# PlayVoice/whisper-vits-svc

Hardware: AMD Instinct MI355X
Metric: audio-seconds/sec end-to-end SVC @32kHz, 10s clips (Whisper-PPG -> flow -> NSF-BigVGAN) (higher is better)
Workload: dtype f32; 1 GPU; configs[1]: batch=1 x 10s clip per GPU, whisper-large-v2 dims (24 of 32 encoder blocks) + base.yaml prior/flow/NSF-BigVGAN; Whisper fp32, synthesizer fp32; clips_in_flight=4, gemm_ring2_mask=12, world_size=1, rccl_ranks_seen=1, whisper_weights_wire=f32, weights=packed on this rank

## Files before the change

whisper-vits-svc_amd/csrc/amp_fused.hip:

```cpp
#include "svcmi_rt.h"
#include "../../include/svcmi.h"

namespace {

constexpr int TPB = 256;
constexpr int RT = 8;
constexpr int CO = 10;
constexpr int DMAX = 5;

#include "snake_math.h"

template <int CP>
__device__ __forceinline__ int tile_row_offset(int t) {
    static_assert(CP == 12 || CP == 20 || CP == 40, "widths of the fused kernels");
    return CP == 12 ? (t << 3) + (t << 2) : CP == 20 ? (t << 4) + (t << 2) : (t << 5) + (t << 3);
}
__device__ __forceinline__ const float* tile_column(const float* xc) {
#ifndef SVCMI_EMU
    asm("" : "+v"(xc));
#endif
    return xc;
}
template <int CP>
__device__ __forceinline__ float tile_x(const float* xc, int t, int n, int ld) {
// ... 7 lines not shown
static inline bool tile_len_ok(int len, int ld) { return (long long)len * ld < (1LL << 31); }

struct AmpArgs {
    const float* x; const float* w; const float* bias; const float* res; float* y;
    const float* alpha_log; const float* beta_log; const float* filt;
    int n, ld, ldw, dil, accumulate, ks;
    float alpha;
};

template <bool H16, int LS>
__device__ __forceinline__ void tile_store(float* S, int row, int ch, float v) {
    if constexpr (H16) reinterpret_cast<unsigned short*>(S)[row * LS + ch] = (unsigned short)svcmi_cvt_pk_f16(v, 0.f);
    else S[row * LS + ch] = v;
}

template <int CP, int CR, int LS, bool H16 = false>
__device__ __forceinline__ void snake_tile(float* S, const float* xb, const float* alpha_log, const float* beta_log,
                                           const float* filt, int n, int ld, int t_blk, int halo, int rows, int tid) {
    struct { const float* alpha_log; const float* beta_log; const float* filt; } p = {alpha_log, beta_log, filt};
        float f[12];
#pragma unroll
        for (int k = 0; k < 12; ++k) f[k] = p.filt[k];
        const int runs = (rows + RT - 1) / RT;
        for (int item = tid; item < runs * CP; item += TPB) {
            const int ch = item % CP, run = item / CP;
            const int r0 = run * RT;
            const int t0 = t_blk - halo + r0;
            float out[RT];
            if (ch >= CR || t0 + RT <= 0 || t0 >= n) {
#pragma unroll
                for (int r = 0; r < RT; ++r) out[r] = 0.f;
            } else {
                const float a = expf(p.alpha_log[ch]);
                const float inv_b = 1.0f / (expf(p.beta_log[ch]) + 1e-9f);
                const float* xc = tile_column(xb + ch);
                SnakeWindow<RT + 10> xw;
#pragma unroll
                for (int i = 0; i < RT + 10; ++i) xw.set(i, tile_x<CP>(xc, t0 - 5 + i, n, ld));
                snake_run<RT>(xw, f, a, inv_b, xc, ld, n, t0, out);
#pragma unroll
                for (int r = 0; r < RT; ++r) {
                    const int t = t0 + r;
                    if (t < 0 || t >= n) out[r] = 0.f;
                }
            }
#pragma unroll
            for (int r = 0; r < RT; ++r)
                if (r0 + r < rows) tile_store<H16, LS>(S, r0 + r, ch, out[r]);
        }
}

template <int CP>
struct UTile {
    static constexpr int LU = 2 * CP + 2;
    __device__ __forceinline__ static int pos(int m) { return m * LU; }
    static constexpr int floats(int pair_rows) { return (pair_rows + 7) * LU; }
};

template <int CP, int CR, int LS, int MAXI, bool H16 = false>
__device__ __forceinline__ void snake_tile_u(float* smem, const float* xb, const float* alpha_log, const float* beta_log,
                                             const float* filt, int n, int ld, int t_blk, int halo, int rows, int tid) {
    constexpr int LU = UTile<CP>::LU;
    float f[12];
#pragma unroll
    for (int k = 0; k < 12; ++k) f[k] = filt[k];
    const int t_lo = t_blk - halo;
    const int pairs = rows + 5;
    const int mruns = (pairs + RT - 1) / RT;
    for (int item = tid; item < mruns * CP; item += TPB) {
        const int ch = item % CP, run = item / CP;
        if (ch >= CR) continue;
        const int m0 = run * RT, tq0 = t_lo + m0;
        svcmi_f32x2 s2[RT];
        if (2 * tq0 - 5 + 2 * RT - 1 < -12 || 2 * tq0 - 5 > 2 * n - 1 + 12) {
#pragma unroll
            for (int m = 0; m < RT; ++m) s2[m] = svcmi_splat2(0.f);
        } else {
            const float a = expf(alpha_log[ch]);
            const float inv_b = 1.0f / (expf(beta_log[ch]) + 1e-9f);
            const float* xc = tile_column(xb + ch);
            SnakeWindow<RT + 5> xw;
#pragma unroll
            for (int i = 0; i < RT + 5; ++i) xw.set(i, tile_x<CP>(xc, tq0 - 5 + i, n, ld));
            snake_pairs<RT>(xw, f, a, inv_b, xc, ld, n, tq0, s2);
        }
#pragma unroll
        for (int m = 0; m < RT; ++m)
            if (m0 + m < pairs) *reinterpret_cast<float2*>(smem + UTile<CP>::pos(m0 + m) + 2 * ch) = make_float2(s2[m][0], s2[m][1]);
    }
    __syncthreads();
    const int runs = (rows + RT - 1) / RT;
    float outs[MAXI][RT];
#pragma unroll
    for (int q = 0; q < MAXI; ++q) {
        const int item = tid + q * TPB;
        if (item < runs * CP) {
            const int ch = item % CP, run = item / CP, r0 = run * RT, t0 = t_lo + r0;
            if (ch >= CR || t0 + RT <= 0 || t0 >= n) {
#pragma unroll
                for (int r = 0; r < RT; ++r) outs[q][r] = 0.f;
            } else {
                svcmi_f32x2 P[RT + 5];
                const float* ub = smem + UTile<CP>::pos(r0) + 2 * ch;
#pragma unroll
                for (int i = 0; i < RT + 5; ++i) {
                    const float2 v = *reinterpret_cast<const float2*>(ub + i * LU);
                    P[i] = svcmi_f32x2{v.x, v.y};
                }
                snake_fir<RT>(P, f, outs[q]);
#pragma unroll
                for (int r = 0; r < RT; ++r) {
                    const int t = t0 + r;
                    if (t < 0 || t >= n) outs[q][r] = 0.f;
                }
            }
        }
    }
    __syncthreads();
#pragma unroll
    for (int q = 0; q < MAXI; ++q) {
        const int item = tid + q * TPB;
        if (item < runs * CP) {
            const int ch = item % CP, r0 = (item / CP) * RT;
#pragma unroll
            for (int r = 0; r < RT; ++r)
                if (r0 + r < rows) tile_store<H16, LS>(smem, r0 + r, ch, outs[q][r]);
        }
    }
}

template <int CP, int G, int TT, int KS>
struct AmpTile {
    static constexpr int TSUB = 4 / G;
    static constexpr int TB = TSUB * 64 * TT;
    static constexpr int LS = (CP / 4) % 2 ? CP : CP + 4;
    static constexpr int ROWS = TB + (KS - 1) * DMAX;
};

template <int CP, int CR, int KS_T, int G, int TT, bool UT = false>
__device__ __forceinline__ void snake_conv_body(const AmpArgs& p, float* S) {
    using TL = AmpTile<CP, G, TT, KS_T ? KS_T : 11>;
    const int KS = KS_T ? KS_T : p.ks;
    constexpr int TSUB = TL::TSUB, TB = TL::TB, LS = TL::LS;
    static_assert(G * CO >= CR && CP % 4 == 0 && CP >= CR, "channel split");

    const int tid = threadIdx.x, lane = tid & 63;
    const int wave = SVCMI_UNIFORM((int)(tid >> 6));
    const int b = blockIdx.y;
    const int n = p.n, ld = p.ld, d = p.dil;
    const int halo = (KS - 1) * d / 2;
    const int t_blk = blockIdx.x * TB;
    const int rows = TB + 2 * halo;
    const float* xb = p.x + (long long)b * n * ld;

    if constexpr (UT) snake_tile_u<CP, CR, LS, (((TL::ROWS + RT - 1) / RT) * CP + TPB - 1) / TPB>(S, xb, p.alpha_log, p.beta_log, p.filt, n, ld, t_blk, halo, rows, tid);
    else snake_tile<CP, CR, LS>(S, xb, p.alpha_log, p.beta_log, p.filt, n, ld, t_blk, halo, rows, tid);
    __syncthreads();

    const int g = wave % G, tsub = wave / G;
// ... 49 lines not shown
                }
            }
        }
    }

    float* yb = p.y + (long long)b * n * ld;
#pragma unroll
    for (int j = 0; j < TT; ++j) {
        const int t = t_blk + tl0 + 64 * j;
        if (t >= n) continue;
        float* yr = yb + (long long)t * ld + co0;
#pragma unroll
        for (int c = 0; c < NCO; c += 2) {
            float v0 = acc[j][c / 2][0], v1 = acc[j][c / 2][1];
            if (co0 + c >= CR) { v0 = 0.f; v1 = 0.f; }
            else {
                if (rb) {
                    float2 r2;
                    if constexpr (PRE) r2 = rpre[j][c / 2];
                    else r2 = *reinterpret_cast<const float2*>(rb + (long long)t * ld + co0 + c);
                    v0 += r2.x; v1 += r2.y;
                }
                v0 *= p.alpha; v1 *= p.alpha;
                if (p.accumulate) { const float2 o2 = *reinterpret_cast<const float2*>(yr + c); v0 += o2.x; v1 += o2.y; }
            }
            *reinterpret_cast<float2*>(yr + c) = make_float2(v0, v1);
        }
        if (g == G - 1) {
#pragma unroll
            for (int c = G * CO; c < CP; c += 2) *reinterpret_cast<float2*>(yb + (long long)t * ld + c) = make_float2(0.f, 0.f);
        }
    }
}

template <int CP, int CR, int KS, int G, int TT>
__global__ __launch_bounds__(TPB) void snake_conv_kernel(AmpArgs p) {
    using TL = AmpTile<CP, G, TT, KS>;
    __shared__ __attribute__((aligned(16))) float S[TL::ROWS * TL::LS];
    snake_conv_body<CP, CR, KS, G, TT>(p, S);
}

constexpr int AMP_GROUP = 3;
struct AmpGroupArgs {
    AmpArgs p[AMP_GROUP];
};

template <int CP, int CR, int G, int TT>
__global__ __launch_bounds__(TPB) void snake_conv_group_kernel(AmpGroupArgs g) {
    using TL = AmpTile<CP, G, TT, 11>;
    __shared__ __attribute__((aligned(16))) float S[TL::ROWS * TL::LS];
    snake_conv_body<CP, CR, 0, G, TT>(g.p[blockIdx.z], S);
}

template <int CP, int CR, int G, int TT>
__global__ __launch_bounds__(TPB) void snake_conv_group_u_kernel(AmpGroupArgs g) {
    using TL = AmpTile<CP, G, TT, 11>;
    constexpr int NU = UTile<CP>::floats(TL::ROWS + 5), NS = TL::ROWS * TL::LS;
    static_assert(((TL::ROWS + RT - 1) / RT) * CP <= 4 * TPB, "snake_tile_u keeps at most 4 work items per thread in registers");
    __shared__ __attribute__((aligned(16))) float S[NU > NS ? NU : NS];
    snake_conv_body<CP, CR, 0, G, TT, true>(g.p[blockIdx.z], S);
}

template <int CP, int CR, int TERMS>
struct Amp16 {
    static constexpr int CK = (CR + 7) / 8;
    static constexpr int LSH = 24;
    static constexpr int NCT = (CR + 15) / 16;
    static constexpr int TB = 256;
    static constexpr int ROWS = TB + 10 * DMAX;
    static constexpr int MAXSTEPS = (11 * CK + 3) / 4;
    static constexpr int S_FLOATS = (ROWS * LSH / 2 + 3) / 4 * 4;
    static constexpr int U_FLOATS = (UTile<CP>::floats(ROWS + 5) + 3) / 4 * 4;
    static constexpr int W_FLOATS = MAXSTEPS * NCT * TERMS * 64 * 4;
    static_assert(CK * 8 <= LSH && CP <= CK * 8 && CP + 4 >= CK * 8, "pad columns [CP, 8 CK) are one 8-byte store per row");
};

template <int CP, int CR, int TERMS, bool UT>
__device__ __forceinline__ void snake_conv16_body(const AmpArgs& p, float* smem, float* wl) {
    using TL = Amp16<CP, CR, TERMS>;
    constexpr int CK = TL::CK, LSH = TL::LSH, NCT = TL::NCT, TB = TL::TB;
    const int KS = p.ks;
    const int tid = threadIdx.x, lane = tid & 63;
    const int wave = SVCMI_UNIFORM((int)(tid >> 6));
    const int b = blockIdx.y;
    const int n = p.n, ld = p.ld, d = p.dil;
    const int halo = (KS - 1) * d / 2;
    const int t_blk = blockIdx.x * TB;
    const int rows = TB + 2 * halo;
    const float* xb = p.x + (long long)b * n * ld;
    const int nsteps = (KS * CK + 3) / 4;

    svcmi_u32x4* wf = reinterpret_cast<svcmi_u32x4*>(wl);
    auto pack_weights = [&] {
    for (int u = tid; u < nsteps * NCT * 64; u += TPB) {
        const int l = u & 63, f = u >> 6;
        const int ct = f % NCT, step = f / NCT;
        const int co = ct * 16 + (l & 15), s = 4 * step + (l >> 4);
        const int tap = s / CK, cb = s - tap * CK;
        float v[8];
#pragma unroll
        for (int h = 0; h < 2; ++h) {
            const int ci0 = cb * 8 + 4 * h;
            float4 q = make_float4(0.f, 0.f, 0.f, 0.f);
            if (co < CR && tap < KS && ci0 < CR) q = *reinterpret_cast<const float4*>(p.w + (long long)co * p.ldw + tap * CP + ci0);
            v[4 * h] = q.x;
            v[4 * h + 1] = ci0 + 1 < CR ? q.y : 0.f;
            v[4 * h + 2] = ci0 + 2 < CR ? q.z : 0.f;
            v[4 * h + 3] = ci0 + 3 < CR ? q.w : 0.f;
// ... 544 lines not shown
```

whisper-vits-svc_amd/csrc/conv_gemm_body.h:

```cpp
#pragma once
#include <type_traits>

#include "svcmi_rt.h"
#include "../../include/svcmi.h"

namespace {

#ifndef SVCMI_GEMM_MIDBAR
#define SVCMI_GEMM_MIDBAR 1
#endif
#ifndef SVCMI_GEMM_SPREAD
#define SVCMI_GEMM_SPREAD 1
#endif
#ifndef SVCMI_PROBE_NOMFMA
#define SVCMI_PROBE_NOMFMA 0
#endif
#ifndef SVCMI_PROBE_KTRACE
#define SVCMI_PROBE_KTRACE 0
#endif
#if SVCMI_PROBE_KTRACE
#ifndef SVCMI_PROBE_KTRACE_N
#define SVCMI_PROBE_KTRACE_N 0
#endif
constexpr unsigned TL_CAP = 1u << 22;
__device__ unsigned long long g_tl[5ull * TL_CAP];
__device__ unsigned g_tl_n;
__device__ unsigned long long g_ktrace[4 * 4 * 8192 + 8];
#endif
#ifndef SVCMI_GEMM_SPREAD2
#define SVCMI_GEMM_SPREAD2 1
#endif
constexpr int BK = 32;
enum { MODE_CHUNK = 0, MODE_VEC = 1, MODE_SCALAR = 2, MODE_CHUNK_RS = 3 };

enum { PREC_F32 = 0, PREC_BF16X3 = 1, PREC_BF16 = 2, PREC_F16 = 3, PREC_BF16_A16 = 4, PREC_F16_A16 = 5, PREC_BF16X3_A16 = 6, PREC_F16W2_A16 = 9 };

struct ConvArgs {
    const float* x; const float* w; const float* bias; const float* res; float* y; const int32_t* lengths;
    float* ws;
    int* cnt;
    long long x_bs, y_bs, r_bs;
    int t_in, t_out, c_in, ldx, n_out, ldw, ldy, ldr;
    int ksize, stride, dil, pad, rshift, act, flags;
    const unsigned short* w16;
    int ldw16;
    unsigned short* y16;
    long long y16_bs;
    int ldy16, y16_f16;
    int vec;
    int ktot;
    int split;
    int mt, nt;
    unsigned magic;
    float alpha;
};

__device__ __forceinline__ float act_apply(float v, int act) {
    switch (act) {
        case SVCMI_ACT_RELU: return v > 0.f ? v : 0.f;
        case SVCMI_ACT_GELU: return svcmi_gelu(v);
        case SVCMI_ACT_MISH: {
            float sp = v;
            if (!(v > 20.f)) {
                const float e = expf(v), u = 1.0f + e;
                sp = u == 1.0f ? e : logf(u) * (e / (u - 1.0f));
            }
            return v * tanhf(sp);
        }
        case SVCMI_ACT_TANH: return tanhf(v);
        case SVCMI_ACT_SIGMOID: return 1.0f / (1.0f + expf(-v));
        default: return v;
    }
}

__device__ __forceinline__ float epilogue(const ConvArgs& p, float v, float bias, const float* res_row, float* dst,
                                          int n, bool masked) {
    v = act_apply(v + bias, p.act);
    if (res_row) v += res_row[n];
    v *= p.alpha;
    if (p.flags & SVCMI_CONV_ACCUMULATE) v += *dst;
    return masked ? 0.f : v;
}

__device__ __forceinline__ int div_magic(int q, unsigned magic) {
    return magic ? (int)__umulhi((unsigned)q, magic) : q;
}

__device__ __forceinline__ int swz(int row) { return (row >> 1) & 7; }
__device__ __forceinline__ int swz16(int row) { return (0x78 >> (((row >> 2) & 3) * 2)) & 3; }

constexpr unsigned OOB = 0x40000000u;

template <int WM, int WN, int MODE, bool P16, int NSTO = 0, int PREC = PREC_F32, int NW = 4>
__device__ __forceinline__ void conv_gemm_body(const ConvArgs& p, const int grid_blocks, const int block_id) {
    static_assert(NW == 4 || (NW == 8 && P16 && PREC == PREC_F32), "eight-wave blocks: fp32 16x16x4 policy only");
    constexpr int NT = 64 * NW;
    constexpr bool A16 = PREC >= PREC_BF16_A16;
    constexpr bool LP = PREC != PREC_F32 && !A16;
    constexpr int KS = A16 ? 2 * BK : BK;
    constexpr unsigned ESZ = A16 ? 2u : 4u;
    constexpr bool F16OP = PREC == PREC_F16 || PREC == PREC_F16_A16 || PREC == PREC_F16W2_A16;
    constexpr bool X3A = PREC == PREC_BF16X3_A16;
    constexpr bool W2A = PREC == PREC_F16W2_A16;
    constexpr int NB = (PREC == PREC_BF16X3 || X3A || W2A) ? 2 : 1;
    constexpr int NA = X3A ? 2 : 1;
    constexpr int BM = P16 ? 16 * WM * NW : 64 * WM, BN = P16 ? 16 * WN : 64 * WN;
    constexpr int BROW = LP ? BK / 2 : BK;
    constexpr int BNL = LP ? (BN + 63) / 64 * 64 : (BN + 8 * NW - 1) / (8 * NW) * (8 * NW);
    constexpr int A_PER = BM / (8 * NW), B_PER = LP ? BNL / 64 : BNL / (8 * NW);
    constexpr int BTILE = BNL * BROW;
    constexpr int CLD = BN;
    constexpr int NST = NSTO ? NSTO : NW == 8 ? 3 : (X3A || (W2A && P16)) ? 2 : (LP ? 3 : (P16 ? ((BM + BNL) > 192 ? 2 : 3) : ((WM * WN == 1) ? 3 : (WM * WN == 2 ? 3 : 2))));
    constexpr int RING = NST * (NA * BM * BK + NB * BTILE);
    static_assert(LP || A16 || BM * CLD <= RING, "C tile must fit in the operand buffers");
    constexpr int BIAS0 = (RING > BM * CLD ? RING : BM * CLD) + 4, BIASN = (BN + 63) / 64 * 64;
    __shared__ __attribute__((aligned(16))) float smem[BIAS0 + BIASN];
    float* const As0 = smem;
    float* const Bs0 = smem + NST * NA * BM * BK;

#if SVCMI_PROBE_KTRACE
    unsigned long long kt_entry, tl_entry;
    asm volatile("s_memtime %0\n\ts_memrealtime %1\n\ts_waitcnt lgkmcnt(0)" : "=s"(kt_entry), "=s"(tl_entry));
#endif
    const int tid = threadIdx.x, lane = tid & 63;
    const int wave = SVCMI_UNIFORM((int)(tid >> 6));
    const int wm = P16 ? wave : (wave >> 1), wn = P16 ? 0 : (wave & 1);
    int bx, by, bz;
    {
        const int total = grid_blocks, id = block_id;
        const int q8 = total >> 3, r8 = total & 7, xcd = id & 7, slot = id >> 3;
        const int L = (xcd < r8 ? xcd * (q8 + 1) : r8 * (q8 + 1) + (xcd - r8) * q8) + slot;
        bx = L % p.mt;
        const int rest = L / p.mt;
        by = rest % p.nt;
        bz = rest / p.nt;
    }
    const int b = bz / p.split, slice = bz - b * p.split;
    const int m0 = bx * BM, n0 = by * BN;
    const int len = p.lengths ? p.lengths[b] : 0x7fffffff;
    const int t_lim = (p.flags & SVCMI_CONV_MASK_IN) ? (len < p.t_in ? len : p.t_in) : p.t_in;
    const int x_rows = (t_lim + (1 << p.rshift) - 1) >> p.rshift;
    const svcmi_rsrc xr = A16 ? svcmi_make_rsrc(reinterpret_cast<const unsigned short*>(p.x) + (long long)b * p.x_bs, (unsigned)x_rows * (unsigned)p.ldx * 2u)
                              : svcmi_make_rsrc(p.x + (long long)b * p.x_bs, (unsigned)x_rows * (unsigned)p.ldx * 4u);
    const svcmi_rsrc wr = (LP || A16) ? svcmi_make_rsrc(p.w16, (unsigned)p.n_out * (unsigned)(NB * p.ldw16) * 2u)
                             : svcmi_make_rsrc(p.w, (unsigned)p.n_out * (unsigned)p.ldw * 4u);

    const int nk_all = (p.ktot + KS - 1) / KS;
    const int it_beg = (int)((long long)nk_all * slice / p.split);
    const int it_end = (int)((long long)nk_all * (slice + 1) / p.split);

    const int prow = lane >> 3;
    const int lkq = ((lane & 7) ^ swz(prow + 8 * wave)) * 4;
    int a_tb[A_PER];
    unsigned a_row[A_PER];
    unsigned b_row[B_PER];
#pragma unroll
    for (int i = 0; i < A_PER; ++i) {
        const int t = m0 + (wave + NW * i) * 8 + prow;
        a_tb[i] = t * p.stride - p.pad;
        a_row[i] = t < p.t_out ? (unsigned)a_tb[i] * (unsigned)p.ldx * ESZ : OOB;
        if (t >= p.t_out) a_tb[i] = -0x40000000;
    }
#pragma unroll
    for (int i = 0; i < B_PER; ++i) {
        const int nl = (wave + NW * i) * (LP ? 16 : 8) + (LP ? (lane >> 2) : prow), n = n0 + nl;
        b_row[i] = (n < p.n_out && nl < BN) ? ((LP || A16) ? (unsigned)(n * NB * p.ldw16) * 2u : (unsigned)(n * p.ldw) * 4u) : OOB;
    }
    const int lkq16 = ((lane & 3) ^ swz16(lane >> 2)) * 16;
    int tap_u = 0, ci_u = 0;
// ... 95 lines not shown
#pragma unroll
        for (int i = 1; i < FA; ++i) svcmi_lds_landed(a4[i]);
#pragma unroll
        for (int j = 0; j < FB; ++j) svcmi_lds_landed(b4[j]);
    };
    auto load_frags_lp = [&](const float* Ab, const float* Bb, int s, svcmi_f32x4 (&a8)[WM][2], svcmi_f32x4 (&b8)[NB][WN], svcmi_f32x4& tie) {
        const int q = (P16 ? 0 : 2 * s) + fhi;
        const int pa = (q ^ swz(frow)) << 2, pb = (q ^ swz16(frow)) << 2;
#pragma unroll
        for (int i = 0; i < WM; ++i) {
            svcmi_lds_read16(a8[i][0], Ab + i * FR * BK + pa, tie);
            svcmi_lds_read16(a8[i][1], Ab + i * FR * BK + (pa ^ 16), tie);
        }
#pragma unroll
        for (int h = 0; h < NB; ++h)
#pragma unroll
            for (int j = 0; j < WN; ++j) svcmi_lds_read16(b8[h][j], Bb + h * BTILE + j * FR * BROW + pb, tie);
    };
    auto frags_arrive_lp = [&](svcmi_f32x4 (&a8)[WM][2], svcmi_f32x4 (&b8)[NB][WN]) {
        svcmi_lds_arrive(a8[0][0]);
        svcmi_lds_landed(a8[0][1]);
#pragma unroll
        for (int i = 1; i < WM; ++i) { svcmi_lds_landed(a8[i][0]); svcmi_lds_landed(a8[i][1]); }
#pragma unroll
        for (int h = 0; h < NB; ++h)
#pragma unroll
            for (int j = 0; j < WN; ++j) svcmi_lds_landed(b8[h][j]);
    };
    auto round_frag = [&](const svcmi_f32x4 (&r)[2], svcmi_u32x4& hi, svcmi_u32x4& lo) {
#pragma unroll
        for (int e = 0; e < 4; ++e) {
            const float x0 = r[e >> 1][2 * (e & 1)], x1 = r[e >> 1][2 * (e & 1) + 1];
            if constexpr (F16OP) {
                hi[e] = svcmi_cvt_pk_f16(x0, x1);
            } else {
                const unsigned h = svcmi_cvt_pk_bf16(x0, x1);
                hi[e] = h;
                if constexpr (NB == 2)
                    lo[e] = svcmi_cvt_pk_bf16(x0 - svcmi_bits_f32(h << 16), x1 - svcmi_bits_f32(h & 0xffff0000u));
            }
        }
    };
    auto mma16 = [&](acc_t& c, svcmi_u32x4 a, svcmi_u32x4 b) {
        if constexpr (P16) c = svcmi_mfma16_16x16x32<F16OP>(a, b, c);
        else c = svcmi_mfma16_32x32x16<F16OP>(a, b, c);
    };

    constexpr int NSUB = LP ? (P16 ? 1 : 2) : (P16 ? BK / 16 : BK / 8);
    constexpr int APCS = NA * A_PER;
    constexpr int PIECES = APCS + NB * B_PER;
    constexpr int DMAS = (MODE == MODE_SCALAR ? 4 * A_PER : APCS) + NB * B_PER;
    constexpr bool MIDBAR = SVCMI_GEMM_MIDBAR != 0 && !LP && !A16;
    constexpr bool SPREAD = SVCMI_GEMM_SPREAD != 0 && MIDBAR && MODE != MODE_SCALAR;
    if (wave < BIASN / 64) {
        const int n = n0 + 64 * wave + lane;
        const svcmi_rsrc br = svcmi_make_rsrc(p.bias, p.bias ? (unsigned)p.n_out * 4u : 0u);
        svcmi_bdma4(p.bias && n < p.n_out ? (unsigned)n * 4u : OOB, svcmi_lds_advance(svcmi_lds_addr(smem + BIAS0), 64 * wave), br);
    }
#pragma unroll
    for (int s0 = 0; s0 < (MIDBAR ? NST : NST - 1); ++s0) {
        if (it_beg + s0 < it_end) {
            stage_prep(it_beg + s0);
#pragma unroll
            for (int i = 0; i < APCS; ++i) stage_a(it_beg + s0, s0, i);
#pragma unroll
            for (int i = 0; i < NB * B_PER; ++i) stage_b(s0, i);
        }
    }
    auto k_step = [&](int it, int slot, int inflight, auto issue_tag) {
        constexpr bool ISSUE = decltype(issue_tag)::value;
        if (ISSUE || inflight == NST - 2) svcmi_dma_wait_n<(NST - 2) * DMAS>();
        else if (inflight == 0) svcmi_dma_wait_n<0>();
        else if (inflight == 1) svcmi_dma_wait_n<DMAS>();
        else svcmi_dma_wait_n<2 * DMAS>();
        __syncthreads();
        int nslot = slot + NST - 1;
        if (nslot >= NST) nslot -= NST;
        if (ISSUE) stage_prep(it + NST - 1);
        const float* Ab = As0 + slot * NA * BM * BK + a_off;
        const float* Bb = Bs0 + slot * NB * BTILE + b_off;
        svcmi_f32x4 tie0 = {0.f, 0.f, 0.f, 0.f};
        if constexpr (LP) {
            svcmi_f32x4 a8[2][WM][2], b8[2][NB][WN];
            load_frags_lp(Ab, Bb, 0, a8[0], b8[0], tie0);
            frags_arrive_lp(a8[0], b8[0]);
#pragma unroll
            for (int s = 0; s < NSUB; ++s) {
                if (s + 1 < NSUB) load_frags_lp(Ab, Bb, s + 1, a8[(s + 1) & 1], b8[(s + 1) & 1], a8[s & 1][0][0]);
                if (ISSUE) {
#pragma unroll
                    for (int q = s * PIECES / NSUB; q < (s + 1) * PIECES / NSUB; ++q) {
                        if (q < A_PER) stage_a(it + NST - 1, nslot, q);
                        else stage_b(nslot, q - A_PER);
                    }
                }
                svcmi_u32x4 ahi[WM], alo[WM];
#pragma unroll
                for (int i = 0; i < WM; ++i) round_frag(a8[s & 1][i], ahi[i], alo[i]);
#pragma unroll
                for (int i = 0; i < WM; ++i)
#pragma unroll
                    for (int j = 0; j < WN; ++j) mma16(acc[i][j], ahi[i], svcmi_as_u32x4(b8[s & 1][0][j]));
                if constexpr (NB == 2) {
#pragma unroll
                    for (int i = 0; i < WM; ++i)
#pragma unroll
                        for (int j = 0; j < WN; ++j) mma16(acc[i][j], alo[i], svcmi_as_u32x4(b8[s & 1][0][j]));
// ... 280 lines not shown
            for (; it + 1 < it_end; advance()) step(it, slot, nxt(), std::true_type(), std::false_type(), std::false_type());
            step(it, slot, nxt(), std::false_type(), std::false_type(), std::false_type());
            }
        }
    } else {
        int it = it_beg, slot = 0;
        for (; it + NST - 1 < it_end; ++it) {
            k_step(it, slot, NST - 2, std::true_type());
            if (++slot == NST) slot = 0;
        }
        for (; it < it_end; ++it) {
            const int rem = it_end - 1 - it;
            k_step(it, slot, rem < NST - 2 ? rem : NST - 2, std::false_type());
            if (++slot == NST) slot = 0;
        }
    }
    svcmi_dma_wait();
    __syncthreads();
#if SVCMI_PROBE_KTRACE
    const bool kt_on = SVCMI_PROBE_KTRACE_N == 0 || p.n_out == SVCMI_PROBE_KTRACE_N;
    if (kt_on && lane == 0 && block_id < 8192 && wave < 4) {
        unsigned long long* kt = g_ktrace + 4 * (block_id * 4 + wave);
        kt[0] = kt_step; kt[1] = kt_vm; kt[2] = kt_bar; kt[3] = kt_n;
        if (block_id == 0 && wave == 0) { g_ktrace[4 * 4 * 8192] = kt_prev - kt_first; g_ktrace[4 * 4 * 8192 + 1] = kt_r1 - kt_r0; g_ktrace[4 * 4 * 8192 + 2] = kt_first - kt_entry; }
    }
    unsigned long long kt_a, kt_b = 0;
    asm volatile("s_memtime %0\n\ts_waitcnt lgkmcnt(0)" : "=s"(kt_a)::"memory");
    auto kt_finish = [&] {
        if (tid == 0) {
            unsigned long long te;
            asm volatile("s_waitcnt vmcnt(0)\n\ts_memrealtime %0\n\ts_waitcnt lgkmcnt(0)" : "=s"(te)::"memory");
            const unsigned idx = atomicAdd(&g_tl_n, 1u);
            if (idx < TL_CAP) {
                unsigned long long* r = g_tl + 5ull * idx;
                r[0] = tl_entry; r[1] = te; r[2] = (unsigned long long)(size_t)p.y ^ ((unsigned long long)(size_t)p.ws << 1);
                r[3] = ((unsigned long long)(unsigned)p.n_out << 32) | (unsigned)p.ktot; r[4] = ((unsigned long long)(unsigned)grid_blocks << 32) | (unsigned)p.t_out;
            }
        }
        if (kt_on && block_id == 0 && tid == 0) {
            unsigned long long t, tc;
            asm volatile("s_memtime %1\n\ts_waitcnt vmcnt(0)\n\ts_memtime %0\n\ts_waitcnt lgkmcnt(0)" : "=s"(t), "=s"(tc)::"memory");
            g_ktrace[4 * 4 * 8192 + 3] = t - kt_prev;
            g_ktrace[4 * 4 * 8192 + 4] += 1;
            g_ktrace[4 * 4 * 8192 + 5] = kt_a - kt_prev;
            g_ktrace[4 * 4 * 8192 + 6] = kt_b - kt_a;
            g_ktrace[4 * 4 * 8192 + 7] = tc - kt_b;
        }
    };
#else
    auto kt_finish = [] {};
#endif

    float* Cs = smem;
#pragma unroll
    for (int i = 0; i < WM; ++i)
#pragma unroll
        for (int j = 0; j < WN; ++j)
#pragma unroll
            for (int r = 0; r < ACC_N; ++r) {
                const int ml = P16 ? (wm * 16 * WM + i * 16 + 4 * (lane >> 4) + r)
                                   : (wm * 32 * WM + i * 32 + (r & 3) + 8 * (r >> 2) + 4 * (lane >> 5));
                const int nl = P16 ? (j * 16 + (lane & 15)) : (wn * 32 * WN + j * 32 + (lane & 31));
                Cs[ml * CLD + nl] = acc[i][j][r];
            }
    __syncthreads();
#if SVCMI_PROBE_KTRACE
    asm volatile("s_memtime %0\n\ts_waitcnt lgkmcnt(0)" : "=s"(kt_b)::"memory");
#endif
    const int nvalid = (p.n_out - n0) < BN ? (p.n_out - n0) : BN;
    const int mvalid = (p.t_out - m0) < BM ? (p.t_out - m0) : BM;
    if (p.split > 1 || (p.flags & SVCMI_CONV_PARTIALS)) {
        float* wsb = p.ws + ((long long)b * p.split + slice) * p.t_out * p.n_out;
        if (!p.cnt) {
            if (p.vec) {
                for (int e = tid; e < BM * (BN / 4); e += NT) {
                    const int ml = e / (BN / 4), nl = (e - ml * (BN / 4)) * 4;
                    if (ml < mvalid && nl < nvalid)
                        *reinterpret_cast<float4*>(wsb + (long long)(m0 + ml) * p.n_out + n0 + nl) = *reinterpret_cast<const float4*>(Cs + ml * CLD + nl);
                }
                kt_finish();
                return;
            }
            for (int e = tid; e < BM * BN; e += NT) {
                const int ml = e / BN, nl = e - ml * BN;
                if (ml < mvalid && nl < nvalid) wsb[(long long)(m0 + ml) * p.n_out + n0 + nl] = Cs[ml * CLD + nl];
            }
            kt_finish();
            return;
        }
        {
            const svcmi_rsrc sr = svcmi_make_rsrc(wsb, (unsigned)p.t_out * (unsigned)p.n_out * 4u);
            for (int e = tid; e < BM * BN / 4; e += NT) {
                const int ml = e / (BN / 4), nl = (e - ml * (BN / 4)) * 4;
                if (ml < mvalid && nl < nvalid)
                    svcmi_store16_sc1(*reinterpret_cast<const svcmi_f32x4*>(Cs + ml * CLD + nl), sr,
                                      (unsigned)((m0 + ml) * p.n_out + n0 + nl) * 4u);
            }
        }
        svcmi_dma_wait();
        __syncthreads();
        int* const flag = reinterpret_cast<int*>(smem + BM * CLD);
        const int tile_id = (b * p.nt + by) * p.mt + bx;
        if (tid == 0) *flag = svcmi_ticket(p.cnt + tile_id);
        __syncthreads();
        if (*flag != p.split - 1) { kt_finish(); return; }
        if (tid == 0) {
            SVCMI_ACQUIRE_AGENT();
            p.cnt[tile_id] = 0;
        }
        __syncthreads();
        float* yb2 = p.y + (long long)b * p.y_bs;
        const float* rb2 = p.res ? p.res + (long long)b * p.r_bs : nullptr;
        const float* ws0 = p.ws + (long long)b * p.split * p.t_out * p.n_out;
        const long long sstride = (long long)p.t_out * p.n_out;
        for (int e = tid; e < BM * BN; e += NT) {
            const int ml = e / BN, nl = e - ml * BN;
            if (ml >= mvalid || nl >= nvalid) continue;
            const int t = m0 + ml, n = n0 + nl;
            const float* src = ws0 + (long long)t * p.n_out + n;
            float v = 0.f;
            for (int sl = 0; sl < p.split; ++sl) v += src[sl * sstride];
            float* dst = yb2 + (long long)t * p.ldy + n;
            *dst = epilogue(p, v, smem[BIAS0 + nl], rb2 ? rb2 + (long long)t * p.ldr : nullptr, dst, n,
                            (p.flags & SVCMI_CONV_MASK_OUT) && t >= len);
        }
        kt_finish();
        return;
    }
    float* yb = p.y + (long long)b * p.y_bs;
    const float* rbp = p.res ? p.res + (long long)b * p.r_bs : nullptr;
    const bool mask_out = (p.flags & SVCMI_CONV_MASK_OUT) != 0;
    if (p.vec) {
        const bool acc_on = (p.flags & SVCMI_CONV_ACCUMULATE) != 0;
        constexpr int EP_IT = BM * (BN / 4) / NT;
        static_assert(BM * (BN / 4) % NT == 0, "whole epilogue iterations");
        constexpr unsigned NOWHERE = 0x80000000u;
        const svcmi_brsrc ry = svcmi_make_brsrc(yb + (long long)m0 * p.ldy + n0, 0x7fffffffu);
        const svcmi_brsrc rr = svcmi_make_brsrc(rbp ? rbp + (long long)m0 * p.ldr + n0 : nullptr, rbp ? 0x7fffffffu : 0u);
        auto loop = [&](auto act_tag, auto loads_tag) {
            constexpr int ACT = decltype(act_tag)::value;
            constexpr bool LOADS = decltype(loads_tag)::value;
            svcmi_f32x4 rv_n = {0.f, 0.f, 0.f, 0.f}, yo_n = {0.f, 0.f, 0.f, 0.f};
            auto where = [&](int e, unsigned& oy, unsigned& orr) {
                const int ml = e / (BN / 4), nl = (e - ml * (BN / 4)) * 4;
                const bool ok = ml < mvalid && nl < nvalid;
                oy = ok ? (unsigned)(ml * p.ldy + nl) * 4u : NOWHERE;
                orr = ok ? (unsigned)(ml * p.ldr + nl) * 4u : NOWHERE;
            };
            unsigned oy_n, or_n;
            where(tid, oy_n, or_n);
            if constexpr (LOADS) {
                rv_n = svcmi_buf_load16(rr, or_n);
                yo_n = svcmi_buf_load16(ry, acc_on ? oy_n : NOWHERE);
            }
#pragma nounroll
            for (int i = 0; i < EP_IT; ++i) {
                const int e = tid + NT * i;
                const int ml = e / (BN / 4), nl = (e - ml * (BN / 4)) * 4;
                const unsigned oy = oy_n;
                const svcmi_f32x4 rv = rv_n, yo = yo_n;
                if constexpr (LOADS) {
                    where(e + NT, oy_n, or_n);
                    rv_n = svcmi_buf_load16(rr, or_n);
                    yo_n = svcmi_buf_load16(ry, acc_on ? oy_n : NOWHERE);
                } else {
                    where(e + NT, oy_n, or_n);
                }
                const int t = m0 + ml;
                const float4 c = *reinterpret_cast<const float4*>(Cs + ml * CLD + nl), bs = *reinterpret_cast<const float4*>(smem + BIAS0 + nl);
                const bool masked = mask_out && t >= len;
                const float cv[4] = {c.x, c.y, c.z, c.w}, bv[4] = {bs.x, bs.y, bs.z, bs.w};
                svcmi_f32x4 o;
#pragma unroll
                for (int k = 0; k < 4; ++k) {
                    float q = act_apply(cv[k] + bv[k], ACT);
                    if (LOADS && rbp) q += rv[k];
                    q *= p.alpha;
                    if (LOADS && acc_on) q += yo[k];
                    o[k] = masked ? 0.f : q;
                }
                svcmi_buf_store16(o, ry, oy);
                if (p.y16 && oy != NOWHERE)
                    svcmi_store4_16(p.y16 + (long long)b * p.y16_bs + (long long)t * p.ldy16 + n0 + nl, p.ldy16 >> 1, o[0], o[1], o[2], o[3], p.y16_f16);
            }
        };
        auto by_act = [&](auto loads_tag) {
            switch (p.act) {
                case SVCMI_ACT_NONE: loop(std::integral_constant<int, SVCMI_ACT_NONE>(), loads_tag); break;
                case SVCMI_ACT_RELU: loop(std::integral_constant<int, SVCMI_ACT_RELU>(), loads_tag); break;
                case SVCMI_ACT_GELU: loop(std::integral_constant<int, SVCMI_ACT_GELU>(), loads_tag); break;
                case SVCMI_ACT_MISH: loop(std::integral_constant<int, SVCMI_ACT_MISH>(), loads_tag); break;
                case SVCMI_ACT_TANH: loop(std::integral_constant<int, SVCMI_ACT_TANH>(), loads_tag); break;
                default: loop(std::integral_constant<int, SVCMI_ACT_SIGMOID>(), loads_tag); break;
            }
        };
        if (rbp || acc_on) by_act(std::true_type());
        else by_act(std::false_type());
        kt_finish();
        return;
    }
    for (int e = tid; e < BM * BN; e += NT) {
        const int ml = e / BN, nl = e - ml * BN;
        if (ml >= mvalid || nl >= nvalid) continue;
        const int t = m0 + ml, n = n0 + nl;
        float* dst = yb + (long long)t * p.ldy + n;
        *dst = epilogue(p, Cs[ml * CLD + nl], smem[BIAS0 + nl], rbp ? rbp + (long long)t * p.ldr : nullptr, dst, n,
                        mask_out && t >= len);
    }
    kt_finish();
}

#ifndef SVCMI_GEMM_NST
#define SVCMI_GEMM_NST 0
#endif
template <int WM, int WN, int MODE, bool P16, int PREC = PREC_F32, int NSTO = 0, int NW = 4>
__global__ __launch_bounds__(64 * NW) void conv_gemm_kernel(ConvArgs p) {
    conv_gemm_body<WM, WN, MODE, P16, (NSTO ? NSTO : (PREC == PREC_F32 && WM * WN <= 5 ? SVCMI_GEMM_NST : 0)), PREC, NW>(p, (int)gridDim.x, (int)blockIdx.x);
}

constexpr int GROUP_MAX = 3;
struct GroupArgs {
    ConvArgs p[GROUP_MAX];
    int first[GROUP_MAX + 1];
};

template <int WM, int WN, int MODE, bool P16, int NSTO, int PREC = PREC_F32>
__global__ __launch_bounds__(256) void conv_gemm_group_kernel(GroupArgs g) {
    const int id = (int)blockIdx.x;
    const int gi = id >= g.first[2] ? 2 : (id >= g.first[1] ? 1 : 0);
    conv_gemm_body<WM, WN, MODE, P16, NSTO, PREC>(g.p[gi], g.first[gi + 1] - g.first[gi], id - g.first[gi]);
}

__global__ __launch_bounds__(256) void splitk_reduce_kernel(ConvArgs p, int batch) {
    const long long total = (long long)batch * p.t_out * p.n_out;
    for (long long e = (long long)blockIdx.x * 256 + threadIdx.x; e < total; e += (long long)gridDim.x * 256) {
        const int n = (int)(e % p.n_out);
        const long long bt = e / p.n_out;
        const int t = (int)(bt % p.t_out), b = (int)(bt / p.t_out);
        const float* src = p.ws + ((long long)b * p.split * p.t_out + t) * p.n_out + n;
        float v = 0.f;
        for (int s = 0; s < p.split; ++s) v += src[(long long)s * p.t_out * p.n_out];
        const int len = p.lengths ? p.lengths[b] : 0x7fffffff;
        float* dst = p.y + (long long)b * p.y_bs + (long long)t * p.ldy + n;
        const float* rr = p.res ? p.res + (long long)b * p.r_bs + (long long)t * p.ldr : nullptr;
        *dst = epilogue(p, v, p.bias ? p.bias[n] : 0.f, rr, dst, n, (p.flags & SVCMI_CONV_MASK_OUT) && t >= len);
    }
}

static int g_last_ring = 0;

template <int WM, int WN, bool P16, int PREC = PREC_F32, int NW = 4>
int launch(const ConvArgs& a_in, int batch, int mode, void* stream) {
    constexpr int BM = P16 ? 16 * WM * NW : 64 * WM, BN = P16 ? 16 * WN : 64 * WN;
    ConvArgs a = a_in;
    a.mt = (a.t_out + BM - 1) / BM;
    a.nt = (a.n_out + BN - 1) / BN;
    const long long blocks = (long long)a.mt * a.nt * batch * a.split;
    if (blocks > 0x7fffffffLL) return SVCMI_EUNSUPPORTED;
    dim3 grid((unsigned)blocks);
    constexpr bool HAS_RING2 = PREC == PREC_F32 && WM == 1 && (P16 ? (WN == 3 || WN == 5) : WN == 1);
    if constexpr (NW == 8) {
        if (mode != MODE_CHUNK && mode != MODE_VEC) return SVCMI_EUNSUPPORTED;
        const bool r2 = (a.flags & SVCMI_CONV_RING2) != 0;
        g_last_ring = r2 ? 2 : 3;
        if (mode == MODE_CHUNK) {
            if (r2) SVCMI_LAUNCH((conv_gemm_kernel<WM, WN, MODE_CHUNK, P16, PREC, 2, 8>), grid, dim3(512), 0, stream, a);
            else SVCMI_LAUNCH((conv_gemm_kernel<WM, WN, MODE_CHUNK, P16, PREC, 3, 8>), grid, dim3(512), 0, stream, a);
        } else {
            if (r2) SVCMI_LAUNCH((conv_gemm_kernel<WM, WN, MODE_VEC, P16, PREC, 2, 8>), grid, dim3(512), 0, stream, a);
            else SVCMI_LAUNCH((conv_gemm_kernel<WM, WN, MODE_VEC, P16, PREC, 3, 8>), grid, dim3(512), 0, stream, a);
        }
        int rc8 = SVCMI_LAST_ERROR();
        if (rc8 == 0 && a.split > 1 && !a.cnt && !(a.flags & SVCMI_CONV_PARTIALS)) {
            const long long total = (long long)batch * a.t_out * a.n_out;
            long long nb = (total + 255) / 256;
            if (nb > 2048) nb = 2048;
            SVCMI_LAUNCH(splitk_reduce_kernel, dim3((unsigned)nb), dim3(256), 0, stream, a, batch);
            rc8 = SVCMI_LAST_ERROR();
        }
        return rc8;
    }
    bool ring2 = false;
    if constexpr (HAS_RING2) ring2 = (a.flags & SVCMI_CONV_RING2) && (mode == MODE_CHUNK || mode == MODE_VEC);
    if constexpr (PREC == PREC_F32) g_last_ring = ring2 ? 2 : 3;
    if (ring2) {
        if constexpr (HAS_RING2) {
            if (mode == MODE_CHUNK) SVCMI_LAUNCH((conv_gemm_kernel<WM, WN, MODE_CHUNK, P16, PREC, 2>), grid, dim3(256), 0, stream, a);
            else SVCMI_LAUNCH((conv_gemm_kernel<WM, WN, MODE_VEC, P16, PREC, 2>), grid, dim3(256), 0, stream, a);
        }
    }
    else if (mode == MODE_CHUNK) SVCMI_LAUNCH((conv_gemm_kernel<WM, WN, MODE_CHUNK, P16, PREC>), grid, dim3(256), 0, stream, a);
    else if (mode == MODE_VEC) SVCMI_LAUNCH((conv_gemm_kernel<WM, WN, MODE_VEC, P16, PREC>), grid, dim3(256), 0, stream, a);
    else if constexpr (!P16) {
        if (mode == MODE_CHUNK_RS) {
            if constexpr (PREC < PREC_BF16_A16) SVCMI_LAUNCH((conv_gemm_kernel<WM, WN, MODE_CHUNK_RS, false, PREC>), grid, dim3(256), 0, stream, a);
            else return SVCMI_EUNSUPPORTED;
        } else if constexpr (PREC == PREC_F32) SVCMI_LAUNCH((conv_gemm_kernel<WM, WN, MODE_SCALAR, false>), grid, dim3(256), 0, stream, a);
        else return SVCMI_EUNSUPPORTED;
// ... 96 lines not shown
```

whisper-vits-svc_amd/csrc/svcmi_rt.h:

```cpp
#pragma once

#ifdef SVCMI_EMU
#include "hip_emu.h"
#else
#include <hip/hip_runtime.h>
#include <stdint.h>

typedef float svcmi_f32x16 __attribute__((ext_vector_type(16)));
typedef float svcmi_f32x4 __attribute__((ext_vector_type(4)));
typedef float svcmi_f32x2 __attribute__((ext_vector_type(2)));
__device__ __forceinline__ svcmi_f32x2 svcmi_fma2(svcmi_f32x2 a, svcmi_f32x2 b, svcmi_f32x2 c) { return __builtin_elementwise_fma(a, b, c); }
__device__ __forceinline__ float svcmi_hsum2(svcmi_f32x2 p) {
    float hi = p[1];
#ifndef SVCMI_EMU
    asm("" : "+v"(hi));
#endif
    return p[0] + hi;
}
__device__ __forceinline__ svcmi_f32x2 svcmi_mul2(svcmi_f32x2 a, svcmi_f32x2 b) { return a * b; }
__device__ __forceinline__ svcmi_f32x2 svcmi_splat2(float v) { return svcmi_f32x2{v, v}; }
__device__ __forceinline__ svcmi_f32x2 svcmi_splat_lo(svcmi_f32x2 p) { return __builtin_shufflevector(p, p, 0, 0); }
__device__ __forceinline__ svcmi_f32x2 svcmi_splat_hi(svcmi_f32x2 p) { return __builtin_shufflevector(p, p, 1, 1); }
__device__ __forceinline__ float svcmi_sgpr_const(float v) {
    int i = __builtin_bit_cast(int, v);
// ... 119 lines not shown
    unsigned keep;
    asm volatile("s_mov_b32 %0, m0\n\ts_mov_b32 m0, %2\n\ts_nop 0\n\tbuffer_load_dword %1, %3, 0 offen lds\n\ts_mov_b32 m0, %0"
                 : "=&s"(keep) : "v"(voff), "s"(lds_wave_base), "s"(rsrc) : "memory");
#endif
}
__device__ __forceinline__ void svcmi_dma_wait() { asm volatile("s_waitcnt vmcnt(0)" ::: "memory"); }
template <int N>
__device__ __forceinline__ void svcmi_dma_wait_n() {
    static_assert(N >= 0 && N < 64, "vmcnt is a 6-bit counter");
    asm volatile("s_waitcnt vmcnt(%0)" ::"n"(N) : "memory");
}

__device__ __forceinline__ void svcmi_lds_read16(svcmi_f32x4& dst, const float* p, svcmi_f32x4& tie) {
    if (SVCMI_PROBE_NOLDSREAD) { asm volatile("" : "=v"(dst), "+v"(tie)); return; }
    const unsigned a = (unsigned)(size_t)(const __attribute__((address_space(3))) float*)p;
    asm volatile("ds_read_b128 %0, %2" : "=v"(dst), "+v"(tie) : "v"(a) : "memory");
}
__device__ __forceinline__ void svcmi_lds_read16(svcmi_f32x4& dst, const float* p, svcmi_f32x4& tie, svcmi_f32x4& tie2) {
    if (SVCMI_PROBE_NOLDSREAD) { asm volatile("" : "=v"(dst), "+v"(tie), "+v"(tie2)); return; }
    const unsigned a = (unsigned)(size_t)(const __attribute__((address_space(3))) float*)p;
    asm volatile("ds_read_b128 %0, %3" : "=v"(dst), "+v"(tie), "+v"(tie2) : "v"(a) : "memory");
}
__device__ __forceinline__ void svcmi_lds_arrive(svcmi_f32x4& d) { asm volatile("s_waitcnt lgkmcnt(0)" : "+v"(d)::"memory"); }
__device__ __forceinline__ void svcmi_lds_arrive(svcmi_f32x4& d, svcmi_f32x4& tie) { asm volatile("s_waitcnt lgkmcnt(0)" : "+v"(d), "+v"(tie)::"memory"); }
__device__ __forceinline__ void svcmi_lds_arrive(svcmi_f32x4& d, svcmi_f32x4& tie, svcmi_f32x4& tie2) {
    asm volatile("s_waitcnt lgkmcnt(0)" : "+v"(d), "+v"(tie), "+v"(tie2)::"memory");
}
__device__ __forceinline__ void svcmi_lds_landed(svcmi_f32x4& d) { asm volatile("" : "+v"(d)::"memory"); }

#ifdef SVCMI_ACC_IN_VGPRS
__device__ __forceinline__ void svcmi_pin(svcmi_f32x16& v) { asm volatile("" : "+v"(v)); }
__device__ __forceinline__ void svcmi_pin(svcmi_f32x4& v) { asm volatile("" : "+v"(v)); }
#else
__device__ __forceinline__ void svcmi_pin(svcmi_f32x16& v) { asm volatile("" : "+a"(v)); }
__device__ __forceinline__ void svcmi_pin(svcmi_f32x4& v) { asm volatile("" : "+a"(v)); }
#endif

#define SVCMI_RELEASE_AGENT() __builtin_amdgcn_fence(__ATOMIC_RELEASE, "agent")
#define SVCMI_ACQUIRE_AGENT() __builtin_amdgcn_fence(__ATOMIC_ACQUIRE, "agent")
__device__ __forceinline__ int svcmi_ticket(int* counter) {
    return __hip_atomic_fetch_add(counter, 1, __ATOMIC_RELAXED, __HIP_MEMORY_SCOPE_AGENT);
}

__device__ __forceinline__ void svcmi_store16_sc1(svcmi_f32x4 v, svcmi_rsrc r, unsigned byte_off) {
    asm volatile("buffer_store_dwordx4 %0, %1, %2, 0 offen sc1\n\ts_nop 1" ::"v"(v), "v"(byte_off), "s"(r) : "memory");
}

typedef __amdgpu_buffer_rsrc_t svcmi_brsrc;
__device__ __forceinline__ svcmi_brsrc svcmi_make_brsrc(const void* base, unsigned bytes) {
    return __builtin_amdgcn_make_buffer_rsrc(const_cast<void*>(base), 0, (int)bytes, 0x00020000);
}
__device__ __forceinline__ svcmi_f32x4 svcmi_buf_load16(svcmi_brsrc r, unsigned byte_off) {
    return __builtin_bit_cast(svcmi_f32x4, __builtin_amdgcn_raw_buffer_load_b128(r, (int)byte_off, 0, 0));
}
__device__ __forceinline__ void svcmi_buf_store16(svcmi_f32x4 v, svcmi_brsrc r, unsigned byte_off) {
    __builtin_amdgcn_raw_buffer_store_b128(__builtin_bit_cast(svcmi_u32x4, v), r, (int)byte_off, 0, 0);
}

#define SVCMI_SCHED_GROUP(mask, n) __builtin_amdgcn_sched_group_barrier(mask, n, 0)

#define SVCMI_UNIFORM(x) __builtin_amdgcn_readfirstlane(x)

#define SVCMI_LAUNCH(kernel, grid, block, shmem, stream, ...) \
    hipLaunchKernelGGL(kernel, grid, block, shmem, (hipStream_t)(stream), __VA_ARGS__)
#define SVCMI_LAST_ERROR() ((int)hipGetLastError())
#endif

#define SVCMI_WAVE 64

#ifndef SVCMI_EMU
__device__ __forceinline__
#else
static inline
#endif
float svcmi_gelu(float v) {
    const float a = fabsf(v) * 0.70710678118654752440f;
    const float t = a < 4.2f ? a : 4.2f;
    float q = -4.535877815214917e-05f;
    q = fmaf(q, t, 0.0004455065354704857f);
    q = fmaf(q, t, -0.0014894307823851705f);
    q = fmaf(q, t, -0.0007746575865894556f);
    q = fmaf(q, t, 0.028253713622689247f);
    q = fmaf(q, t, -0.14848163723945618f);
    q = fmaf(q, t, -0.9184163808822632f);
    q = fmaf(q, t, -1.6279085874557495f);
    const float h = 0.5f * v * svcmi_exp2(q * t);
    const float fit = v > 0.f ? v - h : h, tail = v > 0.f ? v : -0.f;
    return a >= 4.2f ? tail : fit;
}

#ifndef SVCMI_EMU
__device__ __forceinline__
#else
static inline
#endif
void svcmi_store4_16(unsigned short* dst, int lo_off, float a, float b, float c, float d, int fmt) {
    unsigned* h = reinterpret_cast<unsigned*>(dst);
    if (fmt == 1) {
        h[0] = svcmi_cvt_pk_f16(a, b);
        h[1] = svcmi_cvt_pk_f16(c, d);
        return;
    }
    const unsigned h0 = svcmi_cvt_pk_bf16(a, b), h1 = svcmi_cvt_pk_bf16(c, d);
    h[0] = h0;
    h[1] = h1;
    if (fmt == 2) {
        unsigned* l = reinterpret_cast<unsigned*>(dst + lo_off);
        l[0] = svcmi_cvt_pk_bf16(a - svcmi_bits_f32(h0 << 16), b - svcmi_bits_f32(h0 & 0xffff0000u));
        l[1] = svcmi_cvt_pk_bf16(c - svcmi_bits_f32(h1 << 16), d - svcmi_bits_f32(h1 & 0xffff0000u));
    }
}
static inline int svcmi_fmt16(int format) { return format == 2 ? 0 : format == 3 ? 1 : format == 1 ? 2 : -1; }
static inline bool svcmi_fmt16_row_ok(int format, int ld, int n) { return format == 1 ? (ld % 8 == 0 && ld / 2 >= n) : (ld % 4 == 0 && ld >= n); }

#ifdef SVCMI_EMU
template <int N> static inline int svcmi_dpp_row_shr(int x) { const int l = threadIdx.x & 63; return __shfl(x, (l & 15) >= N ? l - N : l); }
static inline int svcmi_dpp_row_bcast15(int x) { const int l = threadIdx.x & 63, r = l >> 4; return __shfl(x, (r == 1 || r == 3) ? 16 * r - 1 : l); }
static inline int svcmi_dpp_row_bcast31(int x) { const int l = threadIdx.x & 63; return __shfl(x, l >= 32 ? 31 : l); }
static inline int svcmi_dpp_wave_shr1(int x) { const int l = threadIdx.x & 63; return __shfl(x, l > 0 ? l - 1 : l); }
#define SVCMI_DEV static inline
#else
template <int N> __device__ __forceinline__ int svcmi_dpp_row_shr(int x) { return __builtin_amdgcn_update_dpp(x, x, 0x110 + N, 0xf, 0xf, false); }
__device__ __forceinline__ int svcmi_dpp_row_bcast15(int x) { return __builtin_amdgcn_update_dpp(x, x, 0x142, 0xa, 0xf, false); }
__device__ __forceinline__ int svcmi_dpp_row_bcast31(int x) { return __builtin_amdgcn_update_dpp(x, x, 0x143, 0xc, 0xf, false); }
__device__ __forceinline__ int svcmi_dpp_wave_shr1(int x) { return __builtin_amdgcn_update_dpp(x, x, 0x138, 0xf, 0xf, false); }
#define SVCMI_DEV __device__ __forceinline__
#endif
template <class F>
SVCMI_DEV double svcmi_dpp_f64(double v, F move) {
    unsigned long long u;
    memcpy(&u, &v, 8);
    const unsigned lo = (unsigned)move((int)(unsigned)u), hi = (unsigned)move((int)(unsigned)(u >> 32));
    u = ((unsigned long long)hi << 32) | lo;
    memcpy(&v, &u, 8);
    return v;
}
```

Before: 1482 audio-seconds/sec.

## Hold GEMM bias in registers, skew snake U-tile LDS, set waves-per-EU

In the f32 conv-GEMM path, bias values are now loaded per lane into registers through buffer loads and added while the accumulator tile is written to LDS. This drops the LDS bias region and shrinks shared memory, which lets more blocks fit on a CU. For the CP=12 snake U-tile, the row stride becomes unpadded and a skew is added every RT rows, which is meant to cut LDS bank conflicts, and the kernel gets an amdgpu_waves_per_eu hint of 5 to raise occupancy. The risks are higher register pressure from the WN bias registers and possible spills under the waves-per-EU constraint.

Result: slower. 1464 audio-seconds/sec (-1.2%).

```diff
diff --git a/whisper-vits-svc_amd/csrc/amp_fused.hip b/whisper-vits-svc_amd/csrc/amp_fused.hip
--- a/whisper-vits-svc_amd/csrc/amp_fused.hip
+++ b/whisper-vits-svc_amd/csrc/amp_fused.hip
@@ -83,15 +83,15 @@
 
 template <int CP>
 struct UTile {
-    static constexpr int LU = 2 * CP + 2;
-    __device__ __forceinline__ static int pos(int m) { return m * LU; }
-    static constexpr int floats(int pair_rows) { return (pair_rows + 7) * LU; }
+    static constexpr int LU = CP == 12 ? 2 * CP : 2 * CP + 2;
+    static constexpr int SKEW = CP == 12 ? 8 : 0;
+    static constexpr int pos(int m) { return m * LU + (m / RT) * SKEW; }
+    static constexpr int floats(int pair_rows) { return pos((pair_rows - 5 + RT - 1) / RT * RT + 5); }
 };
 
 template <int CP, int CR, int LS, int MAXI, bool H16 = false>
 __device__ __forceinline__ void snake_tile_u(float* smem, const float* xb, const float* alpha_log, const float* beta_log,
                                              const float* filt, int n, int ld, int t_blk, int halo, int rows, int tid) {
-    constexpr int LU = UTile<CP>::LU;
     float f[12];
 #pragma unroll
     for (int k = 0; k < 12; ++k) f[k] = filt[k];
@@ -135,7 +135,7 @@
                 const float* ub = smem + UTile<CP>::pos(r0) + 2 * ch;
 #pragma unroll
                 for (int i = 0; i < RT + 5; ++i) {
-                    const float2 v = *reinterpret_cast<const float2*>(ub + i * LU);
+                    const float2 v = *reinterpret_cast<const float2*>(ub + UTile<CP>::pos(i));
                     P[i] = svcmi_f32x2{v.x, v.y};
                 }
                 snake_fir<RT>(P, f, outs[q]);
@@ -291,8 +291,13 @@
     snake_conv_body<CP, CR, 0, G, TT>(g.p[blockIdx.z], S);
 }
 
+#ifdef SVCMI_EMU
+#define SVCMI_WAVES_PER_SIMD(n)
+#else
+#define SVCMI_WAVES_PER_SIMD(n) __attribute__((amdgpu_waves_per_eu(n)))
+#endif
 template <int CP, int CR, int G, int TT>
-__global__ __launch_bounds__(TPB) void snake_conv_group_u_kernel(AmpGroupArgs g) {
+__global__ __launch_bounds__(TPB) SVCMI_WAVES_PER_SIMD(CP == 12 ? 5 : 1) void snake_conv_group_u_kernel(AmpGroupArgs g) {
     using TL = AmpTile<CP, G, TT, 11>;
     constexpr int NU = UTile<CP>::floats(TL::ROWS + 5), NS = TL::ROWS * TL::LS;
     static_assert(((TL::ROWS + RT - 1) / RT) * CP <= 4 * TPB, "snake_tile_u keeps at most 4 work items per thread in registers");
diff --git a/whisper-vits-svc_amd/csrc/conv_gemm_body.h b/whisper-vits-svc_amd/csrc/conv_gemm_body.h
--- a/whisper-vits-svc_amd/csrc/conv_gemm_body.h
+++ b/whisper-vits-svc_amd/csrc/conv_gemm_body.h
@@ -73,9 +73,9 @@
     }
 }
 
-__device__ __forceinline__ float epilogue(const ConvArgs& p, float v, float bias, const float* res_row, float* dst,
+__device__ __forceinline__ float epilogue(const ConvArgs& p, float v, const float* res_row, float* dst,
                                           int n, bool masked) {
-    v = act_apply(v + bias, p.act);
+    v = act_apply(v, p.act);
     if (res_row) v += res_row[n];
     v *= p.alpha;
     if (p.flags & SVCMI_CONV_ACCUMULATE) v += *dst;
@@ -113,8 +113,9 @@
     constexpr int NST = NSTO ? NSTO : NW == 8 ? 3 : (X3A || (W2A && P16)) ? 2 : (LP ? 3 : (P16 ? ((BM + BNL) > 192 ? 2 : 3) : ((WM * WN == 1) ? 3 : (WM * WN == 2 ? 3 : 2))));
     constexpr int RING = NST * (NA * BM * BK + NB * BTILE);
     static_assert(LP || A16 || BM * CLD <= RING, "C tile must fit in the operand buffers");
+    constexpr bool BREG = PREC == PREC_F32;
     constexpr int BIAS0 = (RING > BM * CLD ? RING : BM * CLD) + 4, BIASN = (BN + 63) / 64 * 64;
-    __shared__ __attribute__((aligned(16))) float smem[BIAS0 + BIASN];
+    __shared__ __attribute__((aligned(16))) float smem[BREG ? BIAS0 - 4 : BIAS0 + BIASN];
     float* const As0 = smem;
     float* const Bs0 = smem + NST * NA * BM * BK;
 
@@ -316,7 +317,15 @@
     constexpr int DMAS = (MODE == MODE_SCALAR ? 4 * A_PER : APCS) + NB * B_PER;
     constexpr bool MIDBAR = SVCMI_GEMM_MIDBAR != 0 && !LP && !A16;
     constexpr bool SPREAD = SVCMI_GEMM_SPREAD != 0 && MIDBAR && MODE != MODE_SCALAR;
-    if (wave < BIASN / 64) {
+    float bias_r[WN];
+    if constexpr (BREG) {
+        const svcmi_brsrc br = svcmi_make_brsrc(p.bias, p.bias ? (unsigned)p.n_out * 4u : 0u);
+#pragma unroll
+        for (int j = 0; j < WN; ++j) {
+            const int nl = P16 ? (j * 16 + (lane & 15)) : (wn * 32 * WN + j * 32 + (lane & 31));
+            bias_r[j] = svcmi_buf_load4(br, (unsigned)(n0 + nl) * 4u);
+        }
+    } else if (wave < BIASN / 64) {
         const int n = n0 + 64 * wave + lane;
         const svcmi_rsrc br = svcmi_make_rsrc(p.bias, p.bias ? (unsigned)p.n_out * 4u : 0u);
         svcmi_bdma4(p.bias && n < p.n_out ? (unsigned)n * 4u : OOB, svcmi_lds_advance(svcmi_lds_addr(smem + BIAS0), 64 * wave), br);
@@ -703,6 +712,7 @@
 #endif
 
     float* Cs = smem;
+    const bool raw_tile = p.split > 1 || (p.flags & SVCMI_CONV_PARTIALS);
 #pragma unroll
     for (int i = 0; i < WM; ++i)
 #pragma unroll
@@ -712,7 +722,8 @@
                 const int ml = P16 ? (wm * 16 * WM + i * 16 + 4 * (lane >> 4) + r)
                                    : (wm * 32 * WM + i * 32 + (r & 3) + 8 * (r >> 2) + 4 * (lane >> 5));
                 const int nl = P16 ? (j * 16 + (lane & 15)) : (wn * 32 * WN + j * 32 + (lane & 31));
-                Cs[ml * CLD + nl] = acc[i][j][r];
+                if constexpr (BREG) Cs[ml * CLD + nl] = raw_tile ? acc[i][j][r] : acc[i][j][r] + bias_r[j];
+                else Cs[ml * CLD + nl] = acc[i][j][r];
             }
     __syncthreads();
 #if SVCMI_PROBE_KTRACE
@@ -720,7 +731,7 @@
 #endif
     const int nvalid = (p.n_out - n0) < BN ? (p.n_out - n0) : BN;
     const int mvalid = (p.t_out - m0) < BM ? (p.t_out - m0) : BM;
-    if (p.split > 1 || (p.flags & SVCMI_CONV_PARTIALS)) {
+    if (raw_tile) {
         float* wsb = p.ws + ((long long)b * p.split + slice) * p.t_out * p.n_out;
         if (!p.cnt) {
             if (p.vec) {
@@ -750,7 +761,7 @@
         }
         svcmi_dma_wait();
         __syncthreads();
-        int* const flag = reinterpret_cast<int*>(smem + BM * CLD);
+        int* const flag = reinterpret_cast<int*>(smem);
         const int tile_id = (b * p.nt + by) * p.mt + bx;
         if (tid == 0) *flag = svcmi_ticket(p.cnt + tile_id);
         __syncthreads();
@@ -772,7 +783,10 @@
             float v = 0.f;
             for (int sl = 0; sl < p.split; ++sl) v += src[sl * sstride];
             float* dst = yb2 + (long long)t * p.ldy + n;
-            *dst = epilogue(p, v, smem[BIAS0 + nl], rb2 ? rb2 + (long long)t * p.ldr : nullptr, dst, n,
+            float bv;
+            if constexpr (BREG) bv = p.bias ? p.bias[n] : 0.f;
+            else bv = smem[BIAS0 + nl];
+            *dst = epilogue(p, v + bv, rb2 ? rb2 + (long long)t * p.ldr : nullptr, dst, n,
                             (p.flags & SVCMI_CONV_MASK_OUT) && t >= len);
         }
         kt_finish();
@@ -818,13 +832,15 @@
                     where(e + NT, oy_n, or_n);
                 }
                 const int t = m0 + ml;
-                const float4 c = *reinterpret_cast<const float4*>(Cs + ml * CLD + nl), bs = *reinterpret_cast<const float4*>(smem + BIAS0 + nl);
+                const float4 c = *reinterpret_cast<const float4*>(Cs + ml * CLD + nl);
+                float4 bs = make_float4(0.f, 0.f, 0.f, 0.f);
+                if constexpr (!BREG) bs = *reinterpret_cast<const float4*>(smem + BIAS0 + nl);
                 const bool masked = mask_out && t >= len;
                 const float cv[4] = {c.x, c.y, c.z, c.w}, bv[4] = {bs.x, bs.y, bs.z, bs.w};
                 svcmi_f32x4 o;
 #pragma unroll
                 for (int k = 0; k < 4; ++k) {
-                    float q = act_apply(cv[k] + bv[k], ACT);
+                    float q = act_apply(BREG ? cv[k] : cv[k] + bv[k], ACT);
                     if (LOADS && rbp) q += rv[k];
                     q *= p.alpha;
                     if (LOADS && acc_on) q += yo[k];
@@ -855,7 +871,9 @@
         if (ml >= mvalid || nl >= nvalid) continue;
         const int t = m0 + ml, n = n0 + nl;
         float* dst = yb + (long long)t * p.ldy + n;
-        *dst = epilogue(p, Cs[ml * CLD + nl], smem[BIAS0 + nl], rbp ? rbp + (long long)t * p.ldr : nullptr, dst, n,
+        float v = Cs[ml * CLD + nl];
+        if constexpr (!BREG) v += smem[BIAS0 + nl];
+        *dst = epilogue(p, v, rbp ? rbp + (long long)t * p.ldr : nullptr, dst, n,
                         mask_out && t >= len);
     }
     kt_finish();
@@ -894,7 +912,7 @@
         const int len = p.lengths ? p.lengths[b] : 0x7fffffff;
         float* dst = p.y + (long long)b * p.y_bs + (long long)t * p.ldy + n;
         const float* rr = p.res ? p.res + (long long)b * p.r_bs + (long long)t * p.ldr : nullptr;
-        *dst = epilogue(p, v, p.bias ? p.bias[n] : 0.f, rr, dst, n, (p.flags & SVCMI_CONV_MASK_OUT) && t >= len);
+        *dst = epilogue(p, v + (p.bias ? p.bias[n] : 0.f), rr, dst, n, (p.flags & SVCMI_CONV_MASK_OUT) && t >= len);
     }
 }
 
diff --git a/whisper-vits-svc_amd/csrc/svcmi_rt.h b/whisper-vits-svc_amd/csrc/svcmi_rt.h
--- a/whisper-vits-svc_amd/csrc/svcmi_rt.h
+++ b/whisper-vits-svc_amd/csrc/svcmi_rt.h
@@ -195,6 +195,9 @@
 }
 __device__ __forceinline__ svcmi_f32x4 svcmi_buf_load16(svcmi_brsrc r, unsigned byte_off) {
     return __builtin_bit_cast(svcmi_f32x4, __builtin_amdgcn_raw_buffer_load_b128(r, (int)byte_off, 0, 0));
+}
+__device__ __forceinline__ float svcmi_buf_load4(svcmi_brsrc r, unsigned byte_off) {
+    return __builtin_bit_cast(float, __builtin_amdgcn_raw_buffer_load_b32(r, (int)byte_off, 0, 0));
 }
 __device__ __forceinline__ void svcmi_buf_store16(svcmi_f32x4 v, svcmi_brsrc r, unsigned byte_off) {
     __builtin_amdgcn_raw_buffer_store_b128(__builtin_bit_cast(svcmi_u32x4, v), r, (int)byte_off, 0, 0);
@@ -261,6 +264,11 @@
 static inline int svcmi_dpp_row_bcast15(int x) { const int l = threadIdx.x & 63, r = l >> 4; return __shfl(x, (r == 1 || r == 3) ? 16 * r - 1 : l); }
 static inline int svcmi_dpp_row_bcast31(int x) { const int l = threadIdx.x & 63; return __shfl(x, l >= 32 ? 31 : l); }
 static inline int svcmi_dpp_wave_shr1(int x) { const int l = threadIdx.x & 63; return __shfl(x, l > 0 ? l - 1 : l); }
+static inline float svcmi_buf_load4(svcmi_brsrc r, unsigned byte_off) {
+    float v = 0.f;
+    if ((unsigned long long)byte_off + 4 <= r.bytes) memcpy(&v, r.base + byte_off, 4);
+    return v;
+}
 #define SVCMI_DEV static inline
 #else
 template <int N> __device__ __forceinline__ int svcmi_dpp_row_shr(int x) { return __builtin_amdgcn_update_dpp(x, x, 0x110 + N, 0xf, 0xf, false); }
```
